# jianzhnie/RLZero

Hardware: AMD Instinct MI355X
Metric: mcts_sims_per_sec (higher is better)
Workload: dtype f32 net (hi + lo f16 operand pairs on the f16 MFMA pipe, f32 accumulation) / f64 tree

## Files before the change

profiles/microbench/delta_resident_phases.py:

```python
import ctypes, os, sys
sys.path.insert(0, os.environ.get('GRAFT_REPO_ROOT', '.'))
import rlzero_amd._hip as H
H.library_path = lambda: os.environ.get('RZ_NETPROF_LIB') or os.path.join(os.path.dirname(os.path.abspath(__file__)), 'librlzero_netprof.so')
import rlzero_amd._build as B
B.needs_build = lambda: False
import numpy as np, torch
from rlzero_amd.engine import HipNetEvaluator, MCTSEngine
from rlzero_amd.games.gomoku.policy_value_net import PolicyValueNet
lib = H.load()
NAMES = [(0, 'leaf + changed cells'), (1, 'distances, requests, ranks'), (3, 'maps, base records'), (4, 'bar'), (5, 'conv1'), (6, 'bar'), (7, 'conv2'),
         (9, 'bar + conv3 + heads'), (10, 'bar'), (11, 'features'), (12, 'bar'), (16, 'value layer'), (17, 'expand + backup'),
         (2, 'sel: root record'), (8, 'sel: root scan / answer'), (13, 'sel: level-0 cell'), (14, 'sel: deeper levels'), (15, 'sel: terminal test + leaf stores'),
         (18, 'selection (rest: hand-over)'), (19, 'wave 1: pre-scan'), (20, 'wave 1: wait behind it')]
sizes = [int(a) for a in sys.argv[1:]] or [1, 256, 512]
for games in sizes:
    torch.manual_seed(0)
    net = PolicyValueNet(15).to('cuda:0')
    ev = HipNetEvaluator(net, 15, 'cuda:0', max_boards=games)
    sims = 800
    eng = MCTSEngine(15, 5, n_games=games, n_playout=sims, device='cuda:0', add_noise=True)
    eng.reset_games()
    assert ev.resident_ok(eng) and ev.resident_delta_ok(eng)
    rng = np.random.default_rng(0)
    for ply in range(6):
        eng.sim_chunk(ev, 40)
        visits = eng.root_visits()
        moves = np.array([int(rng.choice(np.flatnonzero(v > 0))) for v in visits], dtype=np.int32)
        eng.advance(moves)
        eng.step(moves)
    a, b = torch.cuda.Event(enable_timing=True), torch.cuda.Event(enable_timing=True)
    ev.hip.delta_stats(reset=True)
    a.record(); eng.sim_chunk(ev, sims); b.record(); torch.cuda.synchronize()
    st = ev.hip.delta_stats()
    out = (ctypes.c_longlong * 24)()
    assert lib.rz_net_debug_profile(out) == 0
    us = 1e3 * a.elapsed_time(b) / sims
    total = out[23] / sims
    print('%d games, %d simulations: %.2f us per simulation of a game (events, bases included), %d cycles (%.2f GHz); %.2f conv3 / %.2f conv2 tiles, %.2f changed cells per leaf, %d leaves without a base' % (
        games, sims, us, total, total / us / 1e3, st['tiles3'] / max(1, st['delta'] + st['no_base']), st['tiles2'] / max(1, st['delta'] + st['no_base']),
        st['cells'] / max(1, st['delta'] + st['no_base']), st['no_base']))
    print('   ' + '  '.join('%s=%d' % (nm, out[k] / sims) for k, nm in NAMES) + '  prescans=%d' % st['prescans'], flush=True)
    eng.close(); ev.hip.close()
```

rlzero_amd/csrc/rz_delta.h:

```cpp
#ifndef RZ_DELTA_TREE_PRIO
#define RZ_DELTA_TREE_PRIO 1
#endif
#ifndef RZ_DELTA_PRO_PRIO
#define RZ_DELTA_PRO_PRIO 0
#endif
#ifndef RZ_DELTA_PRESCAN
#define RZ_DELTA_PRESCAN 1
#endif

namespace dl {

using sp::f16x4;
using sp::f16x8;
typedef const __attribute__((address_space(3))) f16x8 *lds_frag;
typedef const __attribute__((address_space(3))) uint32_t *lds_u32;
typedef __attribute__((address_space(3))) f16x4 *lds_h4;
typedef __attribute__((address_space(3))) f32x4 *lds_v4;

constexpr int kC1Slots = 128, kC2Slots = 164;
constexpr int kT1 = 4, kT2 = 8, kT3 = 8;
constexpr int kMaxD = 4;
constexpr int P1 = rt::Geo<32>::pos_bytes, P2 = rt::Geo<64>::pos_bytes;
constexpr int kGrid = kRowW * kRowW;
constexpr int kShareFloats = kT3 * 4 * 96;
constexpr int kHeadW = 128 * 6 * 4 + 128 * 4 + 32;
constexpr int kOffC1 = sp::kInPieceBytes, kOffC2 = kOffC1 + kC1Slots * P1, kOffZero = kOffC2 + kC2Slots * P2, kOffHead = kOffZero + P2,
              kOffMap1 = kOffHead + kHeadW, kOffMap2 = kOffMap1 + kGrid * 4, kOffList = kOffMap2 + kGrid * 4,
              kLdsBytes = kOffList + 3 * 128 * 2;
static_assert(kShareFloats * 4 <= kC1Slots * P1, "the shares lie inside conv1's records (dead behind conv2)");
constexpr int kWinSets = rzw::kRadii * rzw::kWords, kWinLds = kWinSets * 8 + kWinSets * 4 + 16;
static_assert(2 * (kLdsBytes + 512 * 4 + 4 * 64 * 4 + 80 + kWinLds + (int)sizeof(rzt::RootPre) + 512) <= 160 * 1024,
              "two workgroups per CU, also of the resident search (value row, K-quarter sums, leaf, window sets, root pre-scan)");
static_assert(kOffC1 % 16 == 0 && kOffZero % 16 == 0 && kOffHead % 16 == 0 && kOffMap1 % 16 == 0, "alignment");

constexpr int kCells = RZ_MAX_BOARD_SIZE * RZ_MAX_BOARD_SIZE;
struct BaseHdr {
    uint64_t stones[2 * RZ_BOARD_WORDS];
    int32_t to_move, valid, pad[2];
};
constexpr size_t kBaseC2 = (size_t)kCells * 128, kBaseV = kBaseC2 + (size_t)kCells * 256, kBaseBytes = kBaseV + (size_t)6 * kCells * 4;

struct DeltaArgs {
    BaseHdr *hdr;
    char *recs;
    const uint8_t *active;
    float *feat32;
    unsigned *stats;
    int mode;
    int bw_rcp;
    const uint64_t *win;
};

__device__ __forceinline__ uint32_t lds_addr(const void *p) {
    return (uint32_t)(uintptr_t)((const __attribute__((address_space(3))) char *)p);
}

constexpr int unit_tiles(int nt) { return nt <= 3 ? nt : (nt + 1) / 2; }
constexpr int units_of(int nt) { return (nt + unit_tiles(nt) - 1) / unit_tiles(nt); }

template <int CIN, int NT, int UT>
__device__ __forceinline__ void read_unit(f16x8 (&b)[UT][2], const uint32_t (&rec)[NT][3], int h, int dy, int c) {
#pragma unroll
    for (int i = 0; i < UT; ++i) {
        const int t = h * UT + i;
        if (t < NT) {
            const uint32_t r = rec[t][dy] + (uint32_t)(c * 64);
            b[i][0] = *(lds_frag)(uintptr_t)r;
            b[i][1] = *(lds_frag)(uintptr_t)(r + CIN * 2);
        }
    }
}
template <int TM, int NT, int UT>
__device__ __forceinline__ void mfma_unit(f32x4 (&acc)[TM][NT], const f16x8 (&a)[TM][2], const f16x8 (&b)[UT][2], int h) {
#pragma unroll
    for (int combo = 0; combo < 3; ++combo)
#pragma unroll
        for (int i = 0; i < UT; ++i) {
            const int t = h * UT + i;
            if (t < NT) {
#pragma unroll
                for (int m = 0; m < TM; ++m)
                    acc[m][t] = __builtin_amdgcn_mfma_f32_16x16x32_f16(a[m][combo == 2], b[i][combo == 1], acc[m][t], 0, 0, 0);
            }
        }
}
template <int NT>
__device__ __forceinline__ void lookup(uint32_t (&rec)[NT][3], lds_u32 map, const int (&pos19)[NT], int dx, int g) {
#pragma unroll
    for (int t = 0; t < NT; ++t)
#pragma unroll
        for (int dy = 0; dy < 3; ++dy) rec[t][dy] = map[pos19[t] + dx + dy * kRowW] + (uint32_t)(g * 16);
}

template <int NT>
__device__ __forceinline__ void conv2_g(lds_u32 map, const int (&pos19)[NT], int lane, const f16x8 (&a2)[9][1][2], f32x4 (&acc)[1][NT]) {
    static_assert(NT <= 4, "one unit per step");
    const int g = lane >> 4;
#pragma unroll
    for (int t = 0; t < NT; ++t) acc[0][t] = f32x4{0.f, 0.f, 0.f, 0.f};
    constexpr int AHEAD = NT <= 2 ? 2 : 1;
    uint32_t rec[3][NT][3];
    f16x8 b[AHEAD + 1][NT][2];
#pragma unroll
    for (int dx = 0; dx < 3; ++dx) lookup<NT>(rec[dx], map, pos19, dx, g);
#pragma unroll
    for (int u = 0; u < AHEAD; ++u) read_unit<32, NT, NT>(b[u], rec[u / 3], 0, u % 3, 0);
#pragma unroll
    for (int u = 0; u < 9; ++u) {
        const int dx = u / 3, dy = u % 3;
        if (u + AHEAD < 9) read_unit<32, NT, NT>(b[(u + AHEAD) % (AHEAD + 1)], rec[(u + AHEAD) / 3], 0, (u + AHEAD) % 3, 0);
        mfma_unit<1, NT, NT>(acc, a2[dy * 3 + dx], b[u % (AHEAD + 1)], 0);
        __builtin_amdgcn_sched_barrier(0);
    }
}

#ifndef RZ_DELTA_RING6_UPTO
#define RZ_DELTA_RING6_UPTO 2
#endif
constexpr int ring3(int nt) { return nt <= RZ_DELTA_RING6_UPTO ? 6 : 3; }
__device__ __forceinline__ void load_a3(f16x8 (&a)[2][2], __amdgpu_buffer_rsrc_t w_rsrc, int lane, int dx, int j) {
    using G = rt::Geo<64>;
    const int c = j / 3, dy = j % 3;
#pragma unroll
    for (int m = 0; m < 2; ++m)
#pragma unroll
        for (int p = 0; p < 2; ++p)
            a[m][p] = sp::load_w(w_rsrc, lane * 16, dx * (G::chunks * 2048) + ((m * G::steps + dy * 3 * G::chunks + c) * 2 + p) * 1024);
}
template <int NT>
__device__ __forceinline__ void conv3_g(lds_u32 map, const uint16_t *list3, const void *wts, int lane, bool sync, f32x4 (&acc)[2][NT]) {
    static_assert(NT <= 6, "two units per step");
    constexpr int R = ring3(NT), H = units_of(NT);
    const int n = lane & 15, g = lane >> 4;
    const __amdgpu_buffer_rsrc_t w_rsrc = __builtin_amdgcn_make_buffer_rsrc(const_cast<void *>(wts), 0, 0x7fffffff, 0x00020000);
    f16x8 a3[R][2][2];
#pragma unroll
    for (int j = 0; j < R - 1; ++j) load_a3(a3[j], w_rsrc, lane, 0, j);
    if (sync) __syncthreads();
    int pos19[NT];
#pragma unroll
    for (int t = 0; t < NT; ++t) pos19[t] = (int)list3[16 * t + n] - 19;
#pragma unroll
    for (int m = 0; m < 2; ++m)
#pragma unroll
        for (int t = 0; t < NT; ++t) acc[m][t] = f32x4{0.f, 0.f, 0.f, 0.f};
    uint32_t rec[NT][3], recn[NT][3];
#ifndef RZ_DELTA_AHEAD3_SMALL
#define RZ_DELTA_AHEAD3_SMALL 1
#endif
    constexpr int UT = unit_tiles(NT), AH = UT <= 2 ? RZ_DELTA_AHEAD3_SMALL : 1, NB = AH + 1;
    static_assert((6 * H) % NB == 0 && AH <= H * 6, "a unit's registers are a constant of the unrolled body");
    f16x8 b[NB][UT][2];
    lookup<NT>(rec, map, pos19, 0, g);
#pragma unroll
    for (int u = 0; u < AH; ++u) read_unit<64, NT, UT>(b[u], rec, u % H, (u / H) % 3, u / H / 3);
#pragma unroll 1
    for (int dx = 0; dx < 3; ++dx) {
        lookup<NT>(recn, map, pos19, dx < 2 ? dx + 1 : 2, g);
#pragma unroll
        for (int u = 0; u < 6 * H; ++u) {
            const int j = u / H, h = u % H;
            if (h == 0) {
                const int jj = j + R - 1, dx2 = jj < 6 ? dx : (dx < 2 ? dx + 1 : 2);
                load_a3(a3[jj % R], w_rsrc, lane, dx2, jj % 6);
            }
            {
                const int v = u + AH;
                if (v < 6 * H) read_unit<64, NT, UT>(b[v % NB], rec, v % H, (v / H) % 3, v / H / 3);
                else read_unit<64, NT, UT>(b[v % NB], recn, (v - 6 * H) % H, ((v - 6 * H) / H) % 3, (v - 6 * H) / H / 3);
            }
            mfma_unit<2, NT, UT>(acc, a3[j % R], b[u % NB], h);
            __builtin_amdgcn_sched_barrier(0);
        }
#pragma unroll
        for (int t = 0; t < NT; ++t)
#pragma unroll
            for (int dy = 0; dy < 3; ++dy) rec[t][dy] = recn[t][dy];
    }
}

template <int T>
__device__ __forceinline__ void reduce_scatter(const float (&vals)[6 * T], float (&out)[6 * T / 4]) {
    float r1[3 * T];
#pragma unroll
    for (int i = 0; i < 3 * T; ++i) {
        const auto sw = __builtin_amdgcn_permlane16_swap(__float_as_uint(vals[i]), __float_as_uint(vals[3 * T + i]), false, false);
        r1[i] = __uint_as_float(sw[0]) + __uint_as_float(sw[1]);
    }
#pragma unroll
    for (int i = 0; i < 3 * T / 2; ++i) {
        const auto sw = __builtin_amdgcn_permlane32_swap(__float_as_uint(r1[i]), __float_as_uint(r1[3 * T / 2 + i]), false, false);
        out[i] = __uint_as_float(sw[0]) + __uint_as_float(sw[1]);
    }
}

template <int NT>
__device__ __forceinline__ void conv2_tiles(lds_u32 map1, lds_u32 map2, const uint16_t *list2, int n2, int lane, int wave, const f16x8 (&a2)[9][1][2],
                                            f32x4 bias2, float k2) {
    const int n = lane & 15, g = lane >> 4;
    int pos19[NT];
#pragma unroll
    for (int t = 0; t < NT; ++t) pos19[t] = (int)list2[16 * t + n] - 19;
    f32x4 acc[1][NT];
    conv2_g<NT>(map1, pos19, lane, a2, acc);
#pragma unroll
    for (int t = 0; t < NT; ++t) {
        if (16 * t + n < n2) {
            const uint32_t rec = map2[pos19[t] + kRowW + 1] + (uint32_t)((16 * wave + 4 * g) * 2);
            float z[4];
#pragma unroll
            for (int j = 0; j < 4; ++j) z[j] = fmaxf(fmaf(acc[0][t][j], k2, bias2[j]), 0.0f);
            f16x4 hi, lo;
            sp::split4(z, hi, lo);
            *(lds_h4)(uintptr_t)rec = hi;
            *(lds_h4)(uintptr_t)(rec + 128) = lo;
        }
    }
}

template <int NT>
__device__ __forceinline__ void conv3_tiles(lds_u32 map2, const uint16_t *list3, const void *wts, int lane, int wave, bool sync,
                                            const char *headw, float k3, float *shares) {
    constexpr int T = NT <= 4 ? 4 : 8;
    const int n = lane & 15, g = lane >> 4;
    float vals[6 * T];
    {
        f32x4 acc[2][NT];
        conv3_g<NT>(map2, list3, wts, lane, sync, acc);
        f32x4 hwr[2][6], b3r[2];
#pragma unroll
        for (int m = 0; m < 2; ++m) {
            const int c0 = 32 * wave + 16 * m + 4 * g;
#pragma unroll
            for (int i = 0; i < 6; ++i) hwr[m][i] = *reinterpret_cast<const f32x4 *>(headw + (c0 * 6 + 4 * i) * 4);
            b3r[m] = *reinterpret_cast<const f32x4 *>(headw + 128 * 6 * 4 + c0 * 4);
        }
#pragma unroll
        for (int t = 0; t < T; ++t) {
            f32x2 v2[3] = {f32x2{0.0f, 0.0f}, f32x2{0.0f, 0.0f}, f32x2{0.0f, 0.0f}};
            if (t < NT) {
#pragma unroll
                for (int m = 0; m < 2; ++m)
#pragma unroll
                    for (int j = 0; j < 4; ++j) {
                        const float hv = fmaxf(fmaf(acc[m][t < NT ? t : 0][j], k3, b3r[m][j]), 0.0f);
#pragma unroll
                        for (int o2 = 0; o2 < 3; ++o2) {
                            const int e = 6 * j + 2 * o2;
                            v2[o2] = __builtin_elementwise_fma(f32x2{hwr[m][e >> 2][e & 3], hwr[m][e >> 2][(e & 3) + 1]}, f32x2{hv, hv}, v2[o2]);
                        }
                    }
            }
#pragma unroll
            for (int o = 0; o < 6; ++o) vals[t * 6 + o] = v2[o >> 1][o & 1];
        }
    }
    float mine[6 * T / 4];
    reduce_scatter<T>(vals, mine);
    const int t0 = (T / 2) * (g & 1) + (T / 4) * (g >> 1);
#pragma unroll
    for (int i = 0; i < 6 * T / 4; ++i)
        if (t0 + i / 6 < NT) shares[((t0 + i / 6) * 4 + wave) * 96 + (i % 6) * 16 + n] = mine[i];
}

struct Leaf {
    f16x4 cell_planes;
    const char *base;
    int dys[kMaxD], dxs[kMaxD];
    _Float16 *dst16;
    float *vdst;
    float *dst32;
    const uint64_t *sets;
    bool deferred, store_head;
};
struct Layers {
    float k1, k2, k3, act1, act2, act3;
    const char *t2p, *t3p;
};
#ifdef RZ_NET_PROFILE
struct Prof { long long acc[24], t; };
#else
struct Prof {};
#endif

__device__ __forceinline__ void init_maps(char *lds, int tid) {
    uint32_t *map1 = reinterpret_cast<uint32_t *>(lds + kOffMap1);
    const uint32_t zaddr = lds_addr(lds + kOffZero);
    for (int i = tid; i < 2 * kGrid; i += 256) map1[i] = zaddr;
    if (tid < 3 * 128 / 2) reinterpret_cast<uint32_t *>(lds + kOffList)[tid] = 19u | (19u << 16);
}

__device__ __forceinline__ int cell_dist(int cy, int cx, int pass, const int (&dys)[kMaxD], const int (&dxs)[kMaxD], int BH, int BW) {
    int dist = 1000;
    if (pass < 0) {
#pragma unroll
        for (int i = 0; i < kMaxD; ++i) {
            const int ady = cy > dys[i] ? cy - dys[i] : dys[i] - cy, adx = cx > dxs[i] ? cx - dxs[i] : dxs[i] - cx;
            const int d = ady > adx ? ady : adx;
            dist = d < dist ? d : dist;
        }
    } else {
        const int y0 = 8 * (pass >> 1), x0 = 8 * (pass & 1);
        const int y1 = (y0 + 8 < BH ? y0 + 8 : BH) - 1, x1 = (x0 + 8 < BW ? x0 + 8 : BW) - 1;
        const int ddy = cy < y0 ? y0 - cy : (cy > y1 ? cy - y1 : 0), ddx = cx < x0 ? x0 - cx : (cx > x1 ? cx - x1 : 0);
        dist = ddy > ddx ? ddy : ddx;
    }
    return dist;
}

constexpr int kOutside = 1 << 30;
__device__ __forceinline__ f32x4 load_rec(__amdgpu_buffer_rsrc_t rsrc, int off) {
    return __builtin_bit_cast(f32x4, __builtin_amdgcn_raw_buffer_load_b128(rsrc, off, 0, 0));
}

__device__ __forceinline__ uint64_t uni64(uint64_t v) {
    return ((uint64_t)(unsigned)__builtin_amdgcn_readfirstlane((int)(v >> 32)) << 32) | (unsigned)__builtin_amdgcn_readfirstlane((int)v);
}

template <bool SETS>
__device__ __forceinline__ int delta_passes(const NetDev &nd, const DeltaArgs &da, char *lds, int tid0, int wave, const Leaf &leaf, const Layers &ly,
                                            f32x4 headv, bool &use_delta, Prof &prof) {
    char *in0 = lds, *c1 = lds + kOffC1, *c2 = lds + kOffC2, *zrec = lds + kOffZero, *headw = lds + kOffHead;
    uint32_t *map1 = reinterpret_cast<uint32_t *>(lds + kOffMap1), *map2 = reinterpret_cast<uint32_t *>(lds + kOffMap2);
    uint16_t *list1 = reinterpret_cast<uint16_t *>(lds + kOffList), *list2 = list1 + 128, *list3 = list2 + 128;
    float *shares = reinterpret_cast<float *>(c1);
    const int mode = da.mode, BH = nd.BH, BW = nd.BW, S = nd.S;
    const float k1 = ly.k1, k2 = ly.k2, k3 = ly.k3, act1 = ly.act1, act2 = ly.act2, act3 = ly.act3;
    const char *t2p = ly.t2p, *t3p = ly.t3p;
    const char *base = leaf.base;
    const f16x4 cell_planes = leaf.cell_planes;
    const int (&dys)[kMaxD] = leaf.dys, (&dxs)[kMaxD] = leaf.dxs;
    _Float16 *dst16 = leaf.dst16;
    float *vdst = leaf.vdst, *dst32 = leaf.dst32;
    const bool deferred = leaf.deferred, store_head = leaf.store_head;
    const uint32_t zaddr = lds_addr(zrec);
    int n_conv3_tiles = 0, n_conv2_tiles = 0;
#ifdef RZ_NET_PROFILE
    long long (&prof_acc)[24] = prof.acc, &prof_t = prof.t;
#endif
    for (int pass = use_delta ? -1 : 0; pass < 4; ++pass) {
        int tid = tid0;
        asm volatile("" : "+v"(tid));
        const int lane = tid & 63, g = lane >> 4;
        const int cy = (tid * da.bw_rcp) >> 16, cx = tid - cy * BW;
        const bool is_cell = tid < S;
        const int mypos = is_cell ? (cy + 1) * kRowW + cx + 1 : 0;
        if (RZ_DELTA_PRO_PRIO) __builtin_amdgcn_s_setprio(RZ_DELTA_PRO_PRIO);
        const int th[5] = {pass < 0 ? 1 : 2, pass < 0 ? 2 : 1, pass < 0 ? 3 : 0, pass < 0 ? 3 : 2, pass < 0 ? 4 : 1};
        bool f[5];
        uint64_t own[5];
        const bool handed = SETS && pass < 0;
        if (handed) {
#pragma unroll
            for (int k = 0; k < 5; ++k) {
                own[k] = uni64(leaf.sets[4 * (th[k] - 1) + wave]);
                f[k] = (own[k] >> lane) & 1ull;
            }
        } else {
            const int dist = cell_dist(cy, cx, pass, dys, dxs, BH, BW);
#pragma unroll
            for (int k = 0; k < 5; ++k) f[k] = is_cell && dist <= th[k];
        }
        const bool g1 = pass < 0 && f[3] && !f[0], g2 = pass < 0 && f[4] && !f[1];
        const __amdgpu_buffer_rsrc_t b_rsrc = __builtin_amdgcn_make_buffer_rsrc(const_cast<char *>(base), 0, kBaseBytes, 0x00020000);
        f32x4 r1[8], r2[16];
        {
            const int o1 = g1 ? tid * 128 : kOutside, o2 = g2 ? (int)kBaseC2 + tid * 256 : kOutside;
#pragma unroll
            for (int i = 0; i < 8; ++i) r1[i] = load_rec(b_rsrc, o1 + 16 * i);
#pragma unroll
            for (int i = 0; i < 16; ++i) r2[i] = load_rec(b_rsrc, o2 + 16 * i);
        }
        float bv[6];
        {
            const int ov = pass < 0 && is_cell && !f[2] ? (int)kBaseV + tid * 4 : kOutside;
#pragma unroll
            for (int o = 0; o < 6; ++o) bv[o] = __builtin_bit_cast(float, __builtin_amdgcn_raw_buffer_load_b32(b_rsrc, ov + o * kCells * 4, 0, 0));
        }
        sp::f16x8 a1[3][2];
        f32x4 bias1[4];
        if (32 * wave < 32 * kT1) {
#pragma unroll
            for (int ky = 0; ky < 3; ++ky)
#pragma unroll
                for (int p_ = 0; p_ < 2; ++p_) a1[ky][p_] = __builtin_bit_cast(sp::f16x8, nd.s1[(ky * 2 + p_) * 64 + lane]);
#pragma unroll
            for (int gg = 0; gg < 4; ++gg) bias1[gg] = *reinterpret_cast<const f32x4 *>(nd.b1 + 8 * gg + 4 * (lane >> 5));
        }
        f32x4 bias2 = *reinterpret_cast<const f32x4 *>(nd.b2 + 16 * wave + 4 * g);
        int rank[5], tot[5];
        if (handed) {
            const int *cnt = reinterpret_cast<const int *>(leaf.sets + kWinSets);
#pragma unroll
            for (int k = 0; k < 5; ++k) {
                int before = 0, all = 0;
#pragma unroll
                for (int w = 0; w < 4; ++w) {
                    const int c = __builtin_amdgcn_readfirstlane(cnt[4 * (th[k] - 1) + w]);
                    all += c;
                    before += w < wave ? c : 0;
                }
                rank[k] = before + (int)__builtin_amdgcn_mbcnt_hi((unsigned)(own[k] >> 32), __builtin_amdgcn_mbcnt_lo((unsigned)own[k], 0u));
                tot[k] = all;
            }
        } else {
            int before[5] = {0, 0, 0, 0, 0}, all[5] = {0, 0, 0, 0, 0};
            unsigned long long own[5] = {0ull, 0ull, 0ull, 0ull, 0ull};
#pragma unroll
            for (int b = 0; b < 4; ++b) {
                const int cell = 64 * b + lane, by = (cell * da.bw_rcp) >> 16, bx = cell - by * BW;
                const int d = cell_dist(by, bx, pass, dys, dxs, BH, BW);
#pragma unroll
                for (int k = 0; k < 5; ++k) {
                    const unsigned long long m = __ballot(cell < S && d <= th[k]);
                    const int c = __popcll(m);
                    all[k] += c;
                    before[k] += b < wave ? c : 0;
                    own[k] = b == wave ? m : own[k];
                }
            }
#pragma unroll
            for (int k = 0; k < 5; ++k) {
                rank[k] = before[k] + (int)__builtin_amdgcn_mbcnt_hi((unsigned)(own[k] >> 32), __builtin_amdgcn_mbcnt_lo((unsigned)own[k], 0u));
                tot[k] = all[k];
            }
        }
        NET_TICK(1);
        if (pass < 0 && (tot[0] > 32 * kT1 || tot[1] > 16 * kT2 || tot[2] > 16 * kT3 || tot[3] > kC1Slots || tot[4] > kC2Slots)) {
            use_delta = false;
            continue;
        }
        uint32_t rec1 = 0, rec2 = 0;
        if (f[3]) {
            rec1 = lds_addr(c1 + rank[3] * P1);
            map1[mypos] = rec1;
        }
        if (f[4]) {
            rec2 = lds_addr(c2 + rank[4] * P2);
            map2[mypos] = rec2;
        }
        if (f[0]) list1[rank[0]] = (uint16_t)mypos;
        if (f[1]) list2[rank[1]] = (uint16_t)mypos;
        if (f[2]) list3[rank[2]] = (uint16_t)mypos;
        if (pass <= 0 && is_cell) *reinterpret_cast<f16x4 *>(in0 + ((cy + 1) * sp::kInCols + (cx + 1)) * 8) = cell_planes;
        if (pass <= 0 && store_head && tid < 226) reinterpret_cast<f32x4 *>(headw)[tid] = headv;
        if (g1) {
#pragma unroll
            for (int i = 0; i < 8; ++i) *(lds_v4)(uintptr_t)(rec1 + 16 * i) = r1[i];
        }
        if (g2) {
#pragma unroll
            for (int i = 0; i < 16; ++i) *(lds_v4)(uintptr_t)(rec2 + 16 * i) = r2[i];
        }
        __builtin_amdgcn_sched_barrier(0);
        f16x8 a2[9][1][2];
        {
            const __amdgpu_buffer_rsrc_t w_rsrc = __builtin_amdgcn_make_buffer_rsrc(const_cast<char *>(t2p), 0, 0x7fffffff, 0x00020000);
#pragma unroll
            for (int tap = 0; tap < 9; ++tap)
#pragma unroll
                for (int p = 0; p < 2; ++p) a2[tap][0][p] = sp::load_w(w_rsrc, lane * 16, (tap * 2 + p) * 1024);
        }
        NET_TICK(3);
        __syncthreads();
        NET_TICK(4);

        if (32 * wave < tot[0]) {
            const int n32 = lane & 31, h = lane >> 5, idx = 32 * wave + n32;
            const int pos = list1[idx];
            const int py = (pos * 3641) >> 16, px = pos - py * kRowW;
            typedef const __attribute__((address_space(3))) f16x4 *lds_half;
            const lds_half q = (lds_half)(in0 + ((py - 1) * sp::kInCols + (px - 1) + 2 * h) * 8);
            sp::f16x8 b1[3];
#pragma unroll
            for (int ky = 0; ky < 3; ++ky) {
                const int o = ky * sp::kInCols;
                const f16x4 lo4 = q[o], hi4 = q[o + 1];
                b1[ky] = __builtin_shufflevector(lo4, hi4, 0, 1, 2, 3, 4, 5, 6, 7);
            }
            sp::f32x16 acc1;
#pragma unroll
            for (int r = 0; r < 16; ++r) acc1[r] = 0.0f;
#pragma unroll
            for (int ky = 0; ky < 3; ++ky)
#pragma unroll
                for (int combo = 0; combo < 3; combo += 2)
                    acc1 = __builtin_amdgcn_mfma_f32_32x32x16_f16(a1[ky][combo == 2], b1[ky], acc1, 0, 0, 0);
            if (idx < tot[0]) {
                const uint32_t rec = map1[pos] + (uint32_t)(4 * h * 2);
#pragma unroll
                for (int gg = 0; gg < 4; ++gg) {
                    float z[4];
#pragma unroll
                    for (int j = 0; j < 4; ++j) z[j] = fmaxf(fmaf(acc1[4 * gg + j], k1, bias1[gg][j] * act1), 0.0f);
                    f16x4 hi, lo;
                    sp::split4(z, hi, lo);
                    *(lds_h4)(uintptr_t)(rec + 8 * gg * 2) = hi;
                    *(lds_h4)(uintptr_t)(rec + 8 * gg * 2 + 64) = lo;
                }
            }
        }
        NET_TICK(5);
        __syncthreads();
        NET_TICK(6);
        if (mode == 1 && f[0]) {
            f32x4 *dstp = reinterpret_cast<f32x4 *>(const_cast<char *>(base) + (size_t)tid * 128);
#pragma unroll
            for (int i = 0; i < 8; ++i) dstp[i] = *(lds_v4)(uintptr_t)(rec1 + 16 * i);
        }

        if (RZ_DELTA_PRO_PRIO) __builtin_amdgcn_s_setprio(0);
        const int nt3 = (tot[2] + 15) >> 4;
        {
            const lds_u32 m1 = (lds_u32)map1, m2 = (lds_u32)map2;
            const int nt2 = (tot[1] + 15) >> 4;
            n_conv2_tiles += nt2;
            for (int t0 = 0; t0 < nt2; t0 += 4) {
                const uint16_t *l2 = list2 + 16 * t0;
                const int left = tot[1] - 16 * t0;
                switch (nt2 - t0) {
                    case 1: conv2_tiles<1>(m1, m2, l2, left, lane, wave, a2, bias2 * act2, k2); break;
                    case 2: conv2_tiles<2>(m1, m2, l2, left, lane, wave, a2, bias2 * act2, k2); break;
                    case 3: conv2_tiles<3>(m1, m2, l2, left, lane, wave, a2, bias2 * act2, k2); break;
                    default: conv2_tiles<4>(m1, m2, l2, left, lane, wave, a2, bias2 * act2, k2); break;
                }
            }
        }
        NET_TICK(7);

        {
            const lds_u32 m2 = (lds_u32)map2;
            n_conv3_tiles += nt3;
            const int first = nt3 <= 6 ? nt3 : 4;
            switch (first) {
                case 0: __syncthreads(); break;
                case 1: conv3_tiles<1>(m2, list3, t3p, lane, wave, true, headw, k3, shares); break;
                case 2: conv3_tiles<2>(m2, list3, t3p, lane, wave, true, headw, k3, shares); break;
                case 3: conv3_tiles<3>(m2, list3, t3p, lane, wave, true, headw, k3, shares); break;
                case 4: conv3_tiles<4>(m2, list3, t3p, lane, wave, true, headw, k3, shares); break;
                case 5: conv3_tiles<5>(m2, list3, t3p, lane, wave, true, headw, k3, shares); break;
                default: conv3_tiles<6>(m2, list3, t3p, lane, wave, true, headw, k3, shares); break;
            }
            if (nt3 == 7) conv3_tiles<3>(m2, list3 + 64, t3p, lane, wave, false, headw, k3, shares + 4 * 4 * 96);
            else if (nt3 >= 8) conv3_tiles<4>(m2, list3 + 64, t3p, lane, wave, false, headw, k3, shares + 4 * 4 * 96);
        }
        NET_TICK(9);
        __syncthreads();
        NET_TICK(10);
        if (mode == 1 && f[1]) {
            f32x4 *dstp = reinterpret_cast<f32x4 *>(const_cast<char *>(base) + kBaseC2 + (size_t)tid * 256);
#pragma unroll
            for (int i = 0; i < 16; ++i) dstp[i] = *(lds_v4)(uintptr_t)(rec2 + 16 * i);
        }

        if (is_cell && (pass < 0 || f[2])) {
            const float *share = shares + (rank[2] >> 4) * 4 * 96 + (rank[2] & 15);
            float *basev = mode == 1 ? reinterpret_cast<float *>(const_cast<char *>(base) + kBaseV) : nullptr;
#pragma unroll
            for (int o = 0; o < 6; ++o) {
                float v;
                if (f[2]) {
                    float s = share[o * 16];
#pragma unroll
                    for (int w = 1; w < 4; ++w) s += share[w * 96 + o * 16];
                    v = fmaxf(s + reinterpret_cast<const float *>(headw + 128 * 7 * 4)[o], 0.0f);
                } else {
                    v = bv[o];
                }
                if (mode == 1) {
                    basev[o * kCells + tid] = v;
                    continue;
                }
                if (dst32) dst32[o * S + tid] = v;
                if (deferred && o >= 4) {
                    vdst[(o - 4) * S + tid] = v;
                } else if (dst16) {
                    const int k = (o < 4 ? o : o - 4) * S + tid;
                    const int step = (o < 4 ? 0 : nd.groups_act) + (k >> 4);
                    const float z = v * act3;
                    const _Float16 zh = (_Float16)z;
                    _Float16 *q = dst16 + (size_t)step * 1024 + (k & 15);
                    q[0] = zh;
                    q[512] = (_Float16)(z - (float)zh);
                }
            }
        }
        if (f[3]) map1[mypos] = zaddr;
        if (f[4]) map2[mypos] = zaddr;
        NET_TICK(11);
        if (pass < 0) break;
        __syncthreads();
    }
    return n_conv3_tiles | (n_conv2_tiles << 16);
}

__device__ __forceinline__ f16x4 planes_of(const uint64_t (&ls)[8], int tid, int tm_eff, bool has_last, int lc, int par_count) {
    f16x4 cell_planes;
    const int word = (tid >> 6) & 3, bit = tid & 63;
    uint64_t w0 = 0ull, w1 = 0ull;
#pragma unroll
    for (int w = 0; w < 4; ++w) {
        const uint64_t mk = word == w ? ~0ull : 0ull;
        w0 |= ls[w] & mk;
        w1 |= ls[4 + w] & mk;
    }
    const bool s0 = (w0 >> bit) & 1ull, s1 = (w1 >> bit) & 1ull;
    const bool mine = tm_eff == 0 ? s0 : s1, theirs = tm_eff == 0 ? s1 : s0;
    const _Float16 one = (_Float16)sp::kObsScale, zero = (_Float16)0.0f;
    cell_planes[0] = mine ? one : zero;
    cell_planes[1] = theirs ? one : zero;
    cell_planes[2] = (has_last && tid == lc) ? one : zero;
    cell_planes[3] = (par_count & 1) ? zero : one;
    return cell_planes;
}

__device__ __forceinline__ bool changed_cells(const uint64_t (&ls)[8], const uint64_t (&rs)[8], int nst, int tm, int lc, bool has_last, bool base_ok, int h_tm,
                                              int bw_rcp, int BW, int (&dys)[kMaxD], int (&dxs)[kMaxD], int &parity, int &nD) {
    bool use_delta = false;
    {
        bool sup = true;
        int nroot = 0;
        uint64_t D[4] = {0ull, 0ull, 0ull, 0ull};
#pragma unroll
        for (int q = 0; q < 8; ++q) {
            sup = sup && (rs[q] & ~ls[q]) == 0ull;
            nroot += __popcll(rs[q]);
            D[q & 3] |= rs[q] ^ ls[q];
        }
#pragma unroll
        for (int w = 0; w < 4; ++w) D[w] |= (has_last && lc >= 0 && (lc >> 6) == w) ? 1ull << (lc & 63) : 0ull;
        parity = (nst - nroot) & 1;
        nD = __popcll(D[0]) + __popcll(D[1]) + __popcll(D[2]) + __popcll(D[3]);
        use_delta = base_ok && sup && tm == (h_tm ^ parity) && nD <= kMaxD;
#pragma unroll
        for (int i = 0; i < kMaxD; ++i) {
            const bool z0 = D[0] == 0ull, z1 = D[1] == 0ull, z2 = D[2] == 0ull;
            const int w = !z0 ? 0 : !z1 ? 1 : !z2 ? 2 : 3;
            const uint64_t word = !z0 ? D[0] : !z1 ? D[1] : !z2 ? D[2] : D[3];
            const bool any = word != 0ull;
            const int cell = 64 * w + __builtin_ctzll(word | (1ull << 63));
            const uint64_t rest = word & (word - 1ull);
#pragma unroll
            for (int k = 0; k < 4; ++k) D[k] = k == w ? rest : D[k];
            const int y = (cell * bw_rcp) >> 16;
            dys[i] = any ? y : -100;
            dxs[i] = any ? cell - y * BW : -100;
        }
    }
    return use_delta;
}

template <bool TRACE>
__global__ __launch_bounds__(256, 2) void k_trunk_delta(NetDev nd, LeafBits leaves, _Float16 *__restrict__ feat16, int n_boards,
                                                        DeferredOut later, DeltaArgs da) {
    __shared__ __attribute__((aligned(16))) char lds[kLdsBytes];
    const int board = blockIdx.x;
    const int mode = da.mode;
    const int game = mode == 1 ? board >> 1 : board, par_b = mode == 1 ? board & 1 : 0;
    unsigned long long trace_t0 = 0;
    if (TRACE) trace_t0 = rz_trace_now();
    Prof prof;
#ifdef RZ_NET_PROFILE
    for (int i = 0; i < 24; ++i) prof.acc[i] = 0;
    prof.t = __builtin_readcyclecounter();
    const long long prof_k0 = prof.t;
    long long (&prof_acc)[24] = prof.acc, &prof_t = prof.t;
#endif
    const int tid0 = threadIdx.x, wave = __builtin_amdgcn_readfirstlane(tid0 >> 6);
    const int BW = nd.BW, S = nd.S;
    Layers ly;
    ly.t2p = reinterpret_cast<const char *>(nd.t2) + (size_t)wave * rt::Geo<32>::steps * 2 * 1024;
    ly.t3p = reinterpret_cast<const char *>(nd.t3) + (size_t)(2 * wave) * rt::Geo<64>::steps * 2 * 1024;
    f32x4 headv = tid0 < 192 ? reinterpret_cast<const f32x4 *>(nd.whp)[tid0] : reinterpret_cast<const f32x4 *>(nd.b3)[(tid0 - 192) & 31];
    {
        const float *bh = nd.bh + (tid0 == 225 ? 4 : 0);
        const f32x4 hbv = {bh[0], bh[1], tid0 == 225 ? 0.0f : bh[2], tid0 == 225 ? 0.0f : bh[3]};
        headv = (tid0 == 224 || tid0 == 225) ? hbv : headv;
    }
    ly.k1 = nd.s_inv[2], ly.k2 = nd.s_inv[0], ly.k3 = nd.s_inv[1];
    ly.act1 = nd.s_inv[5], ly.act2 = nd.s_inv[6], ly.act3 = nd.s_inv[7];

    const uint64_t *sb = leaves.stones + (size_t)game * 8;
    const BaseHdr *hd = da.hdr + game;
    uint64_t ls[8], rs[8];
    int nst = 0;
#pragma unroll
    for (int q = 0; q < 8; ++q) {
        ls[q] = sb[q];
        rs[q] = hd->stones[q];
        nst += __popcll(ls[q]);
    }
    const int tm = leaves.to_move[game];
    const int lc_raw = (mode == 1 ? leaves.to_move : leaves.last)[game];
    const int lc = mode == 1 ? -1 : lc_raw;
    const int h_tm = hd->to_move, h_valid = hd->valid;
    const int is_active = da.active[game];
    const bool deferred = later.slot_of != nullptr;
    const int slot_ = (deferred ? later.slot_of : leaves.to_move)[deferred ? board : game];
    const int tm_eff = tm ^ par_b;
    const int par_count = nst + par_b;
    const bool has_last = mode != 1 && nst > 0;

    Leaf leaf;
    int parity = 0, nD = 0;
    bool use_delta = changed_cells(ls, rs, nst, tm, lc, has_last, mode == 0 && h_valid != 0, h_tm, da.bw_rcp, BW, leaf.dys, leaf.dxs, parity, nD);
    leaf.base = da.recs + ((size_t)game * 2 + (mode == 1 ? par_b : parity)) * kBaseBytes;
    leaf.cell_planes = planes_of(ls, tid0, tm_eff, has_last, lc, par_count);

    leaf.dst16 = nullptr;
    leaf.vdst = nullptr;
    if (mode != 1 && deferred) {
        leaf.dst16 = (feat16 != nullptr && slot_ < later.n_slots) ? feat16 + (size_t)slot_ * later.slot_halfs + (size_t)(board >> 5) * nd.groups_act * 1024 + (board & 31) * 16 : nullptr;
        leaf.vdst = later.valfeat + (size_t)board * later.vf_ld;
    }
    if (mode != 1 && !deferred && feat16 != nullptr)
        leaf.dst16 = feat16 + ((size_t)(board >> 5) * (nd.groups_act + nd.groups_val) * 1024 + (board & 31) * 16);
    leaf.dst32 = (mode != 1 && da.feat32 != nullptr) ? da.feat32 + (size_t)board * 6 * S : nullptr;
    leaf.sets = nullptr;
    leaf.deferred = deferred;
    leaf.store_head = true;

    {
        const f32x4 zero = {0.f, 0.f, 0.f, 0.f};
        f32x4 *z = reinterpret_cast<f32x4 *>(lds);
        for (int i = tid0; i < sp::kInPieceBytes / 16; i += 256) z[i] = zero;
        if (tid0 < P2 / 16) reinterpret_cast<f32x4 *>(lds + kOffZero)[tid0] = zero;
        init_maps(lds, tid0);
    }
    if (mode == 0 && is_active == 0) return;
    __syncthreads();
    NET_TICK(0);
    const int n_tiles = delta_passes<false>(nd, da, lds, tid0, wave, leaf, ly, headv, use_delta, prof);
    const int n_conv3_tiles = n_tiles & 0xffff;

    if (mode == 1 && par_b == 0 && tid0 == 0) {
        BaseHdr *h = da.hdr + game;
#pragma unroll
        for (int q = 0; q < 8; ++q) h->stones[q] = sb[q];
        h->to_move = tm;
        h->valid = 1;
    }
    if (da.stats != nullptr && tid0 == 0 && mode != 1) {
        atomicAdd(da.stats + (use_delta ? 0 : 1), 1u);
        atomicAdd(da.stats + 2, (unsigned)n_conv3_tiles);
        atomicAdd(da.stats + 3, (unsigned)nD);
        atomicAdd(da.stats + 4, (unsigned)(n_tiles >> 16));
    }
#ifdef RZ_NET_PROFILE
    if (blockIdx.x == 0 && tid0 == 0) {
        for (int i = 0; i < 24; ++i) net_prof[i] = prof_acc[i];
        net_prof[23] = __builtin_readcyclecounter() - prof_k0;
        net_prof[22] = n_conv3_tiles;
    }
#endif
    if (TRACE && tid0 == 0) rz_trace_write(later.trace, RZ_TRACE_TRUNK, deferred ? slot_ : 0, board, trace_t0);
}

__device__ __forceinline__ void windows_store(uint64_t row, bool use_delta, int parity, int nD, int lane, uint64_t *ws) {
    unsigned lo = (unsigned)row, hi = (unsigned)(row >> 32);
    {
        const auto a = __builtin_amdgcn_permlane16_swap(lo, lo, false, false), b = __builtin_amdgcn_permlane16_swap(hi, hi, false, false);
        lo = a[0] | a[1];
        hi = b[0] | b[1];
    }
    {
        const auto a = __builtin_amdgcn_permlane32_swap(lo, lo, false, false), b = __builtin_amdgcn_permlane32_swap(hi, hi, false, false);
        lo = a[0] | a[1];
        hi = b[0] | b[1];
    }
    const uint64_t v = ((uint64_t)hi << 32) | lo;
    int *cnt = reinterpret_cast<int *>(ws + kWinSets);
    if (lane < kWinSets) {
        ws[lane] = v;
        cnt[lane] = __popcll(v);
    }
    if (lane == 0) cnt[kWinSets] = (use_delta ? 1 : 0) | (parity << 1) | (nD << 8);
}
__device__ __forceinline__ void leaf_windows(const uint64_t *leaf_lds, const uint64_t (&rs)[8], bool base_ok, int h_tm, const DeltaArgs &da, int BW,
                                             int lane, uint64_t *ws) {
    uint64_t ls[8];
    int nst = 0;
#pragma unroll
    for (int q = 0; q < 8; ++q) {
        ls[q] = uni64(leaf_lds[q]);
        nst += __popcll(ls[q]);
    }
    const int tm = __builtin_amdgcn_readfirstlane(reinterpret_cast<const int *>(leaf_lds + 2 * RZ_BOARD_WORDS)[0]);
    const int lc = __builtin_amdgcn_readfirstlane(reinterpret_cast<const int *>(leaf_lds + 2 * RZ_BOARD_WORDS)[1]);
    int dys[kMaxD], dxs[kMaxD], parity = 0, nD = 0;
    const bool use_delta = changed_cells(ls, rs, nst, tm, lc, nst > 0, base_ok, h_tm, da.bw_rcp, BW, dys, dxs, parity, nD);
    const int i = lane >> 4;
    int dy = dys[0], dx = dxs[0];
#pragma unroll
    for (int j = 1; j < kMaxD; ++j) {
        dy = i == j ? dys[j] : dy;
        dx = i == j ? dxs[j] : dx;
    }
    const bool any = dy >= 0;
    const uint64_t row = da.win[(any ? dy * BW + dx : 0) * kWinSets + (lane & (kWinSets - 1))];
    windows_store(any ? row : 0ull, use_delta, parity, nD, lane, ws);
}

#if defined(RZ_NET_PROFILE) && !defined(RZ_SEL_TICKS)
#define RZ_SEL_TICKS 0
#endif
struct ResHook {
    static constexpr bool kOn = true;
    rzt::RootPre *pre;
    const uint64_t *win;
    int depth;
    bool any0;
    uint64_t row;
    __device__ __forceinline__ void root_cell(int last, int stones, int lane) {
        any0 = stones > 0 && last >= 0 && last < kCells;
        row = win[(any0 ? last : 0) * kWinSets + (lane & (kWinSets - 1))];
    }
    __device__ __forceinline__ void cell(int level, int c, int lane) {
        const uint64_t v = win[c * kWinSets + (lane & (kWinSets - 1))];
        row = (lane >> 4) == level ? v : row;
    }
#ifdef RZ_NET_PROFILE
    Prof *prof;
    __device__ __forceinline__ void tick(int i, int arrived) {
        if ((RZ_SEL_TICKS >> i) & 1) {
            asm volatile("" ::"v"(arrived));
            const int slot = i == 0 ? 2 : i == 1 ? 8 : 12 + i;
            __builtin_amdgcn_sched_barrier(0);
            const long long now = __builtin_readcyclecounter();
            prof->acc[slot] += now - prof->t;
            prof->t = now;
            __builtin_amdgcn_sched_barrier(0);
        }
    }
#else
    __device__ __forceinline__ void tick(int, int) {}
#endif
};

__device__ __forceinline__ void path_windows(const ResHook &hook, bool base_ok, int lane, uint64_t *ws) {
    const int depth = hook.depth;
    const bool mine = depth == 0 ? (lane < 16 && hook.any0) : (lane >> 4) < depth;
    const int nD = depth == 0 ? (hook.any0 ? 1 : 0) : depth;
    windows_store(mine ? hook.row : 0ull, base_ok && nD <= kMaxD, depth & 1, nD, lane, ws);
}

constexpr int kResVrow = 512;
__global__ __launch_bounds__(256, 2) void k_delta_res(NetDev nd, _Float16 *__restrict__ store16, DeferredOut later, DeltaArgs da, ResArgs<true> res) {
    __shared__ __attribute__((aligned(16))) char lds[kLdsBytes];
    __shared__ float res_vrow[kResVrow];
    __shared__ float res_part[rzt::kDefWaves][rzt::kWave];
    __shared__ __attribute__((aligned(16))) uint64_t res_leaf[2 * RZ_BOARD_WORDS + 2];
    __shared__ __attribute__((aligned(16))) uint64_t res_win[kWinLds / 8];
    __shared__ __attribute__((aligned(16))) rzt::RootPre res_pre;
    const int game = blockIdx.x;
    if (game >= res.E.n_games || res.E.active[game] == 0) return;
    const unsigned long long clk0 = __builtin_readcyclecounter(), rt0 = __builtin_amdgcn_s_memrealtime();
    const int tid0 = threadIdx.x, wave = __builtin_amdgcn_readfirstlane(tid0 >> 6);
    const int BW = nd.BW;
    Prof prof;
#ifdef RZ_NET_PROFILE
    for (int i = 0; i < 24; ++i) prof.acc[i] = 0;
    prof.t = __builtin_readcyclecounter();
    const long long prof_k0 = prof.t;
    long long (&prof_acc)[24] = prof.acc, &prof_t = prof.t;
#endif
    Layers ly;
    ly.t2p = reinterpret_cast<const char *>(nd.t2) + (size_t)wave * rt::Geo<32>::steps * 2 * 1024;
    ly.t3p = reinterpret_cast<const char *>(nd.t3) + (size_t)(2 * wave) * rt::Geo<64>::steps * 2 * 1024;
    f32x4 headv = tid0 < 192 ? reinterpret_cast<const f32x4 *>(nd.whp)[tid0] : reinterpret_cast<const f32x4 *>(nd.b3)[(tid0 - 192) & 31];
    {
        const float *bh = nd.bh + (tid0 == 225 ? 4 : 0);
        const f32x4 hbv = {bh[0], bh[1], tid0 == 225 ? 0.0f : bh[2], tid0 == 225 ? 0.0f : bh[3]};
        headv = (tid0 == 224 || tid0 == 225) ? hbv : headv;
    }
    ly.k1 = nd.s_inv[2], ly.k2 = nd.s_inv[0], ly.k3 = nd.s_inv[1];
    ly.act1 = nd.s_inv[5], ly.act2 = nd.s_inv[6], ly.act3 = nd.s_inv[7];
    const int slot0 = res.E.pend[game];
    uint64_t rs[8];
    bool base_ok = da.hdr[game].valid != 0;
#pragma unroll
    for (int q = 0; q < 8; ++q) {
        rs[q] = res.E.root_stones[(size_t)game * 8 + q];
        base_ok = base_ok && da.hdr[game].stones[q] == rs[q];
    }
    const int h_tm = res.E.root_to_move[game];
    base_ok = base_ok && da.hdr[game].to_move == h_tm;
    {
        const f32x4 zero = {0.f, 0.f, 0.f, 0.f};
        f32x4 *z = reinterpret_cast<f32x4 *>(lds);
        for (int i = tid0; i < sp::kInPieceBytes / 16; i += 256) z[i] = zero;
        if (tid0 < P2 / 16) reinterpret_cast<f32x4 *>(lds + kOffZero)[tid0] = zero;
        init_maps(lds, tid0);
        for (int i = tid0; i < kResVrow; i += 256) res_vrow[i] = 0.0f;
    }
    if (tid0 == 0) res_pre.scan = res_pre.valid = res_pre.answered = 0;
    ResHook hook;
    hook.pre = &res_pre;
    hook.win = da.win;
    hook.depth = 0;
    hook.any0 = false;
    hook.row = 0ull;
#ifdef RZ_NET_PROFILE
    hook.prof = &prof;
    long long pre_cycles = 0, pre_wait = 0;
#endif
    if (res.select_first == 0 && tid0 == 0) {
#pragma unroll
        for (int q = 0; q < 8; ++q) res_leaf[q] = res.E.leaf_stones[(size_t)game * 8 + q];
        reinterpret_cast<int *>(res_leaf + 2 * RZ_BOARD_WORDS)[0] = res.E.leaf_to_move[game];
        reinterpret_cast<int *>(res_leaf + 2 * RZ_BOARD_WORDS)[1] = res.E.leaf_last[game];
    }
    __syncthreads();
    if (wave == 0) {
        const int lane0 = tid0 & 63;
        if (res.select_first != 0) {
            rzt::select_body<false, rzt::kWords, ResHook>(res.E, nullptr, game, lane0, 0, res_leaf, &hook);
            path_windows(hook, base_ok, lane0, res_win);
        } else {
            leaf_windows(res_leaf, rs, base_ok, h_tm, da, BW, lane0, res_win);
        }
    }
    __syncthreads();
    int tiles_total = 0, tiles2_total = 0, deltas = 0, cells_total = 0;
    for (int sim = 0; sim < res.n_sims; ++sim) {
        int tid_s = tid0;
        asm volatile("" : "+v"(tid_s));
        uint64_t ls[8];
        int nst = 0;
#pragma unroll
        for (int q = 0; q < 8; ++q) {
            const uint64_t v = res_leaf[q];
            ls[q] = ((uint64_t)(unsigned)__builtin_amdgcn_readfirstlane((int)(v >> 32)) << 32) | (unsigned)__builtin_amdgcn_readfirstlane((int)v);
            nst += __popcll(ls[q]);
        }
        const int tm = __builtin_amdgcn_readfirstlane(reinterpret_cast<const int *>(res_leaf + 2 * RZ_BOARD_WORDS)[0]);
        const int lc = __builtin_amdgcn_readfirstlane(reinterpret_cast<const int *>(res_leaf + 2 * RZ_BOARD_WORDS)[1]);
        const bool has_last = nst > 0;
        const int verdict = __builtin_amdgcn_readfirstlane(reinterpret_cast<const int *>(res_win + kWinSets)[kWinSets]);
        bool use_delta = (verdict & 1) != 0;
        const int parity = (verdict >> 1) & 1, nD = verdict >> 8;
        Leaf leaf;
        leaf.sets = res_win;
#pragma unroll
        for (int i = 0; i < kMaxD; ++i) leaf.dys[i] = leaf.dxs[i] = -100;
        leaf.base = da.recs + ((size_t)game * 2 + parity) * kBaseBytes;
        leaf.cell_planes = planes_of(ls, tid_s, tm, has_last, lc, nst);
        leaf.dst16 = slot0 + sim < later.n_slots ? store16 + (size_t)(slot0 + sim) * later.slot_halfs + (size_t)(game >> 5) * nd.groups_act * 1024 + (game & 31) * 16 : nullptr;
        leaf.vdst = res_vrow;
        leaf.dst32 = nullptr;
        leaf.deferred = true;
        leaf.store_head = sim == 0;
        NET_TICK(0);
        const int n_tiles = delta_passes<true>(nd, da, lds, tid_s, wave, leaf, ly, headv, use_delta, prof);
        tiles_total += n_tiles & 0xffff;
        tiles2_total += n_tiles >> 16;
        deltas += use_delta ? 1 : 0;
        cells_total += nD;
        __syncthreads();
        NET_TICK(12);
        const int lane = tid_s & 63;
        if (RZ_DELTA_TREE_PRIO) __builtin_amdgcn_s_setprio(RZ_DELTA_TREE_PRIO);
        if (res.vh.groups == 128) rzt::value_quarter_lds<16>(res.vh, res_vrow, lane, wave, res_part);
        else rzt::value_quarter_lds<8>(res.vh, res_vrow, lane, wave, res_part);
        NET_TICK(16);
        const bool more = sim + 1 < res.n_sims;
        if (wave == 0) {
            rzt::expand_backup_body<float, false, false, false, true>(res.E, nullptr, nullptr, game, lane, rz_raw_heads(), 0, res.vh, res_part);
        } else {
            __syncthreads();
            if (RZ_DELTA_PRESCAN && wave == 1 && more) {
#ifdef RZ_NET_PROFILE
                const long long t0 = __builtin_readcyclecounter();
#endif
                rzt::root_prescan<rzt::kWords>(res.E, game, lane, &res_pre);
#ifdef RZ_NET_PROFILE
                __builtin_amdgcn_s_waitcnt(0);
                const long long t1 = __builtin_readcyclecounter();
                pre_cycles += t1 - t0;
                pre_wait -= t1;
#endif
            }
        }
        __syncthreads();
#ifdef RZ_NET_PROFILE
        if (RZ_DELTA_PRESCAN && wave == 1 && more) pre_wait += __builtin_readcyclecounter();
#endif
        NET_TICK(17);
        if (wave == 0 && more) {
            hook.depth = 0, hook.any0 = false, hook.row = 0ull;
            int lane_t = lane;
            asm volatile("" : "+v"(lane_t));
            rzt::select_body<false, rzt::kWords, ResHook>(res.E, nullptr, game, lane_t, 0, res_leaf, &hook);
            path_windows(hook, base_ok, lane_t, res_win);
        }
        if (RZ_DELTA_TREE_PRIO) __builtin_amdgcn_s_setprio(0);
        __syncthreads();
        NET_TICK(18);
    }
    if (da.stats != nullptr && tid0 == 0) {
        atomicAdd(da.stats + 0, (unsigned)deltas);
        atomicAdd(da.stats + 1, (unsigned)(res.n_sims - deltas));
        atomicAdd(da.stats + 2, (unsigned)tiles_total);
        atomicAdd(da.stats + 3, (unsigned)cells_total);
        atomicAdd(da.stats + 4, (unsigned)tiles2_total);
        atomicAdd(da.stats + 5, (unsigned)res_pre.answered);
        if (game == 0) {
            da.stats[6] = (unsigned)((__builtin_readcyclecounter() - clk0) >> 8);
            da.stats[7] = (unsigned)(__builtin_amdgcn_s_memrealtime() - rt0);
        }
    }
#ifdef RZ_NET_PROFILE
    if (blockIdx.x == 0 && tid0 == 0) {
        for (int i = 0; i < 24; ++i)
            if (i != 19 && i != 20) net_prof[i] = prof_acc[i];
        net_prof[23] = __builtin_readcyclecounter() - prof_k0;
        net_prof[22] = tiles_total;
    }
    if (blockIdx.x == 0 && tid0 == 64) {
        net_prof[19] = pre_cycles;
        net_prof[20] = pre_wait;
    }
#endif
}

}
```

Measured before the change: 21.43 million.

## Defer policy-plane feature stores to idle waves during expand/backup

In the resident delta kernel, the first four policy output planes are no longer computed and stored inside the delta passes. Waves 2 and 3 now do that work while wave 0 runs expand and backup, rebuilding the values from the LDS shares and the base records using the window bitsets and ranks. The aim is to take work off the critical path of the network phase and place it in otherwise idle waves. The cost is extra buffer loads and LDS reads in that window, plus a dependency on the shares staying valid in LDS until the barrier.

```diff
diff --git a/profiles/microbench/delta_resident_phases.py b/profiles/microbench/delta_resident_phases.py
--- a/profiles/microbench/delta_resident_phases.py
+++ b/profiles/microbench/delta_resident_phases.py
@@ -11,7 +11,8 @@
 NAMES = [(0, 'leaf + changed cells'), (1, 'distances, requests, ranks'), (3, 'maps, base records'), (4, 'bar'), (5, 'conv1'), (6, 'bar'), (7, 'conv2'),
          (9, 'bar + conv3 + heads'), (10, 'bar'), (11, 'features'), (12, 'bar'), (16, 'value layer'), (17, 'expand + backup'),
          (2, 'sel: root record'), (8, 'sel: root scan / answer'), (13, 'sel: level-0 cell'), (14, 'sel: deeper levels'), (15, 'sel: terminal test + leaf stores'),
-         (18, 'selection (rest: hand-over)'), (19, 'wave 1: pre-scan'), (20, 'wave 1: wait behind it')]
+         (18, 'selection (rest: hand-over)'), (19, 'wave 1: pre-scan'), (20, 'wave 1: wait behind it'),
+         (21, 'wave 2: policy pieces'), (22, 'wave 2: wait behind them')]
 sizes = [int(a) for a in sys.argv[1:]] or [1, 256, 512]
 for games in sizes:
     torch.manual_seed(0)
diff --git a/rlzero_amd/csrc/rz_delta.h b/rlzero_amd/csrc/rz_delta.h
--- a/rlzero_amd/csrc/rz_delta.h
+++ b/rlzero_amd/csrc/rz_delta.h
@@ -272,6 +272,7 @@
     float *dst32;
     const uint64_t *sets;
     bool deferred, store_head;
+    bool late = false;
 };
 struct Layers {
     float k1, k2, k3, act1, act2, act3;
@@ -333,6 +334,7 @@
     _Float16 *dst16 = leaf.dst16;
     float *vdst = leaf.vdst, *dst32 = leaf.dst32;
     const bool deferred = leaf.deferred, store_head = leaf.store_head;
+    const bool late = SETS && leaf.late;
     const uint32_t zaddr = lds_addr(zrec);
     int n_conv3_tiles = 0, n_conv2_tiles = 0;
 #ifdef RZ_NET_PROFILE
@@ -375,7 +377,8 @@
         {
             const int ov = pass < 0 && is_cell && !f[2] ? (int)kBaseV + tid * 4 : kOutside;
 #pragma unroll
-            for (int o = 0; o < 6; ++o) bv[o] = __builtin_bit_cast(float, __builtin_amdgcn_raw_buffer_load_b32(b_rsrc, ov + o * kCells * 4, 0, 0));
+            for (int o = 0; o < 6; ++o)
+                bv[o] = late && o < 4 ? 0.0f : __builtin_bit_cast(float, __builtin_amdgcn_raw_buffer_load_b32(b_rsrc, ov + o * kCells * 4, 0, 0));
         }
         sp::f16x8 a1[3][2];
         f32x4 bias1[4];
@@ -558,6 +561,7 @@
             float *basev = mode == 1 ? reinterpret_cast<float *>(const_cast<char *>(base) + kBaseV) : nullptr;
 #pragma unroll
             for (int o = 0; o < 6; ++o) {
+                if (late && pass < 0 && o < 4) continue;
                 float v;
                 if (f[2]) {
                     float s = share[o * 16];
@@ -844,6 +848,63 @@
     windows_store(mine ? hook.row : 0ull, base_ok && nD <= kMaxD, depth & 1, nD, lane, ws);
 }
 
+__device__ __forceinline__ void policy_late(const char *lds, const uint64_t *ws, const char *base, _Float16 *dst16, int S, float act3, int t) {
+    typedef _Float16 f16x8s __attribute__((ext_vector_type(8)));
+    const float *shares = reinterpret_cast<const float *>(lds + kOffC1);
+    const float *hb = reinterpret_cast<const float *>(lds + kOffHead + 128 * 7 * 4);
+    const int *cnt = reinterpret_cast<const int *>(ws + kWinSets);
+    uint64_t w3[4];
+    int before[4];
+    {
+        int c = 0;
+#pragma unroll
+        for (int w = 0; w < 4; ++w) {
+            w3[w] = uni64(ws[8 + w]);
+            before[w] = c;
+            c += __builtin_amdgcn_readfirstlane(cnt[8 + w]);
+        }
+    }
+    const __amdgpu_buffer_rsrc_t b_rsrc = __builtin_amdgcn_make_buffer_rsrc(const_cast<char *>(base), 0, kBaseBytes, 0x00020000);
+    const int k0 = 8 * t, n = 4 * S - k0;
+    float bv[8];
+    int slot[8];
+#pragma unroll
+    for (int j = 0; j < 8; ++j) {
+        const int k = k0 + j;
+        const int o = (k >= S) + (k >= 2 * S) + (k >= 3 * S);
+        const int cell = k - o * S;
+        const int word = (cell >> 6) & 3, bit = cell & 63;
+        const uint64_t m = word == 0 ? w3[0] : word == 1 ? w3[1] : word == 2 ? w3[2] : w3[3];
+        const int bf = word == 0 ? before[0] : word == 1 ? before[1] : word == 2 ? before[2] : before[3];
+        const bool in = j < n && ((m >> bit) & 1ull) != 0ull;
+        const int rank = bf + __popcll(m & ((1ull << bit) - 1ull));
+        slot[j] = in ? (rank >> 4) * 4 * 96 + (rank & 15) + o * 16 : -1;
+        const int ov = j < n && !in ? (int)kBaseV + (o * kCells + cell) * 4 : kOutside;
+        bv[j] = __builtin_bit_cast(float, __builtin_amdgcn_raw_buffer_load_b32(b_rsrc, ov, 0, 0));
+    }
+    f16x8s hi, lo;
+#pragma unroll
+    for (int j = 0; j < 8; ++j) {
+        const bool in = slot[j] >= 0;
+        const float *share = shares + (in ? slot[j] : 0);
+        float s = share[0];
+#pragma unroll
+        for (int w = 1; w < 4; ++w) s += share[w * 96];
+        const float v = in ? fmaxf(s + hb[(slot[j] >> 4) & 3], 0.0f) : bv[j];
+        const float z = v * act3;
+        hi[j] = (_Float16)z;
+        lo[j] = (_Float16)(z - (float)hi[j]);
+    }
+    _Float16 *q = dst16 + (size_t)(k0 >> 4) * 1024 + (k0 & 15);
+    if (n >= 8) {
+        *reinterpret_cast<f16x8s *>(q) = hi;
+        *reinterpret_cast<f16x8s *>(q + 512) = lo;
+    } else if (n > 0) {
+        *reinterpret_cast<f16x4 *>(q) = __builtin_shufflevector(hi, hi, 0, 1, 2, 3);
+        *reinterpret_cast<f16x4 *>(q + 512) = __builtin_shufflevector(lo, lo, 0, 1, 2, 3);
+    }
+}
+
 constexpr int kResVrow = 512;
 __global__ __launch_bounds__(256, 2) void k_delta_res(NetDev nd, _Float16 *__restrict__ store16, DeferredOut later, DeltaArgs da, ResArgs<true> res) {
     __shared__ __attribute__((aligned(16))) char lds[kLdsBytes];
@@ -903,6 +964,7 @@
 #ifdef RZ_NET_PROFILE
     hook.prof = &prof;
     long long pre_cycles = 0, pre_wait = 0;
+    long long late_cycles = 0, late_wait = 0;
 #endif
     if (res.select_first == 0 && tid0 == 0) {
 #pragma unroll
@@ -950,6 +1012,7 @@
         leaf.dst32 = nullptr;
         leaf.deferred = true;
         leaf.store_head = sim == 0;
+        leaf.late = true;
         NET_TICK(0);
         const int n_tiles = delta_passes<true>(nd, da, lds, tid_s, wave, leaf, ly, headv, use_delta, prof);
         tiles_total += n_tiles & 0xffff;
@@ -980,10 +1043,31 @@
                 pre_wait -= t1;
 #endif
             }
+            if (wave >= 2 && use_delta) {
+                __builtin_amdgcn_s_setprio(0);
+#ifdef RZ_NET_PROFILE
+                const long long t0 = __builtin_readcyclecounter();
+#endif
+                const int slot = slot0 + sim;
+                const int par = (__builtin_amdgcn_readfirstlane(reinterpret_cast<const int *>(res_win + kWinSets)[kWinSets]) >> 1) & 1;
+                if (slot < later.n_slots)
+                    policy_late(lds, res_win, da.recs + ((size_t)game * 2 + par) * kBaseBytes,
+                                store16 + (size_t)slot * later.slot_halfs + (size_t)(game >> 5) * nd.groups_act * 1024 + (game & 31) * 16, nd.S, ly.act3,
+                                tid_s - 128);
+#ifdef RZ_NET_PROFILE
+                if (wave == 2) {
+                    __builtin_amdgcn_s_waitcnt(0);
+                    const long long t1 = __builtin_readcyclecounter();
+                    late_cycles += t1 - t0;
+                    late_wait -= t1;
+                }
+#endif
+            }
         }
         __syncthreads();
 #ifdef RZ_NET_PROFILE
         if (RZ_DELTA_PRESCAN && wave == 1 && more) pre_wait += __builtin_readcyclecounter();
+        if (wave == 2 && use_delta) late_wait += __builtin_readcyclecounter();
 #endif
         NET_TICK(17);
         if (wave == 0 && more) {
@@ -1012,15 +1096,18 @@
 #ifdef RZ_NET_PROFILE
     if (blockIdx.x == 0 && tid0 == 0) {
         for (int i = 0; i < 24; ++i)
-            if (i != 19 && i != 20) net_prof[i] = prof_acc[i];
+            if (i < 19 || i > 22) net_prof[i] = prof_acc[i];
         net_prof[23] = __builtin_readcyclecounter() - prof_k0;
-        net_prof[22] = tiles_total;
     }
     if (blockIdx.x == 0 && tid0 == 64) {
         net_prof[19] = pre_cycles;
         net_prof[20] = pre_wait;
     }
-#endif
-}
-
-}
+    if (blockIdx.x == 0 && tid0 == 128) {
+        net_prof[21] = late_cycles;
+        net_prof[22] = late_wait;
+    }
+#endif
+}
+
+}
```

Result: slower. 21.02 million (-1.9%).
